# craftman22/medane_tchakorom_ufc_thesis_repository

Measured on AMD Instinct MI355X. Metric: DOF-updates/s on 3D 7-pt Poisson GMRES; achieved HBM GB/s vs peak, 1/2/4/8 GPU, higher is better.
Workload: dtype f64

## Files before the change

### medane_tchakorom_ufc_thesis_repository_amd/csrc/msplit_kernels.h

```cpp
#pragma once

#include <hip/hip_runtime.h>

#include <cstdint>

#define MSK_MAX_GROUP 32
#define MSK_DBR_CHUNK 4096

enum { MSK_SET = 0, MSK_COPY, MSK_SCALE, MSK_AXPY, MSK_AYPX, MSK_WAXPY_P1, MSK_WAXPY_M1, MSK_WAXPY };

struct Vecs {
  const double* p[MSK_MAX_GROUP];
  const double* base;
  int64_t stride;
  const double* scale;
};
struct Coefs {
  double a[MSK_MAX_GROUP];
};
struct EllOp {
  const uint8_t* code8;
  const int32_t* ddelta;
  const double* dval;
  int ndict;
// ... 11 lines not shown
  MSK_TUNE_SPMV_TEMPORAL = 2,
  MSK_TUNE_SPMV_XCD = 4,
  MSK_TUNE_SPMV_STAGE1 = 8,
  MSK_TUNE_VEC_TEMPORAL = 16,
  MSK_TUNE_MAXPY_TEMPORAL_ST = 64,
  MSK_TUNE_GM_UNFUSED = 128,
  MSK_TUNE_MAXPY_HALVES = 256,
  MSK_TUNE_SPMV_ZCHUNK = 512,
  MSK_TUNE_MDOT_SINGLE = 1024,
  MSK_TUNE_GM_SPMV_MDOT = 2048,
  MSK_TUNE_SPMV_MDOT_G2 = 4096,
  MSK_TUNE_DV_RPL1 = 8192,
  MSK_TUNE_DV_RPL2 = 16384,
  MSK_TUNE_DV_NOELL = 32768,
  MSK_TUNE_GM_OPFUSE = 65536,
  MSK_TUNE_MAXPY_UNROLL1 = 131072,
  MSK_TUNE_MDOT_UNROLL2 = 262144,
  MSK_TUNE_ELL_TEMPORAL_Y = 1048576,
  MSK_TUNE_SPMV_NTY = 2097152,
  MSK_TUNE_SPMV_REG_STAGE = 4194304,
  MSK_TUNE_DENSE_G1 = 8388608,
  MSK_TUNE_DENSE_G2 = 16777216,
  MSK_TUNE_DENSE_TEMPORAL_ST = 33554432,
  MSK_TUNE_ELL_XCD_ON = 67108864,
  MSK_TUNE_ELL_XCD_OFF = 134217728,
  MSK_TUNE_ELL_MARCH_OFF = 268435456,
  MSK_TUNE_ELL_MARCH_NOXCD = 536870912,
  MSK_TUNE_GM_BOX_MDOT_OFF = 1073741824,
  MSK_TUNE_BOX_MDOT_NOXCD = 524288,
  MSK_TUNE_BOX_MDOT_FLAT = 32
};

extern "C" {
void msk_set_tuning(int flags);
int msk_get_tuning(void);
void msk_set_spmv_group(int gb);
void msk_set_march_z(int z);
void msk_set_march_lines(int l);
int msk_dot_stage1_op(const EllOp* op, const Vecs* V, int nv, int64_t n, double* partial, int64_t nchunks,
                      const int* stop, hipStream_t s);
int msk_maxpy_op(const EllOp* op, double* wout, const Vecs* V, int nv, const double* adev, int64_t n,
                 double* partial, const int* stop, hipStream_t s);
int msk_dot_stage1(const double* w, const Vecs* V, int nv, int64_t n, double* partial, int64_t nchunks, int self,
                   const int* stop, hipStream_t s);
int msk_dot_stage2(const double* partial, int64_t nchunks, int nv, double* out, const int* stop, hipStream_t s);
int msk_seq_stage1(const double* w, const Vecs* V, int nv, int64_t n, int self, double* partial, int64_t nchunks,
                   const int* stop, hipStream_t s);
int msk_maxpy_chunk(const double* win, double* wout, const Vecs* V, int nv, const int* nvdev, const Coefs* A,
                    const double* adev, int negate, int64_t n, int accum, double* partial, const int* stop,
                    hipStream_t s);
int msk_maxpy_mdot(const double* win, double* wout, const Vecs* V, int nv, const double* adev, int64_t n,
                   double* partial, int64_t nchunks, const int* stop, hipStream_t s);
int msk_spmv(int32_t nrows, const int32_t* rowptr, const int32_t* col, const double* val, const double* x,
             const double* b, double* y, int32_t lds_cap, int mode, const double* sdev, double* vout,
             const int* stop, int64_t plane, hipStream_t s);
int msk_spmv_dv(int32_t nrows, const int32_t* rowptr, const uint8_t* len8, const uint8_t* code8,
                const int32_t* ddelta, const double* dval, int ndict, int32_t max_block, int ell_w,
                const double* x, const double* b, double* y, int mode, const double* sdev, double* vout,
                const int* stop, int64_t plane, hipStream_t s);
int msk_box_march_pick(int32_t nx, int32_t ny, int32_t nz);
int msk_march_mask(int32_t nrows, int d2, const uint8_t* code8, uint8_t* mask, hipStream_t s);
int msk_march_check(int32_t nrows, int32_t nx, int32_t ny, int d2, const uint8_t* mask, int* fail, hipStream_t s);
int msk_spmv_box_march(int32_t nx, int32_t ny, int32_t nz, int d2, const uint8_t* mask, const double* dval,
                       const double* x, const double* b, double* y, int mode, const double* sdev, double* vout,
                       const int* stop, hipStream_t s);
int msk_march_chunk_fits(int32_t nx, int32_t ny, int d2);
int msk_box_march_halo_fits(int32_t nx, int32_t ny, int32_t nz, int halo, const double *x, const double *b,
                            const double *y, int mode);
int msk_box_march_halo(int32_t nx, int32_t ny, int32_t nz, int halo, const uint8_t* mask, const double* dval,
                       const double* x, const double* b, double* y, int mode, hipStream_t s);
int msk_box_march_chunk_rv(int32_t nx, int32_t ny, int32_t nz, const uint8_t* mask, const double* rv, int64_t rvs,
                           const double* x, const double* b, double* y, int mode, const double* sdev, double* vout,
                           const int* stop, hipStream_t s);
int msk_box_spmv_mdot_rv(int32_t nx, int64_t P, int64_t n, int d2, const uint8_t* mask, const double* dval,
                         const double* rv, int64_t rvs, const double* x, const double* sdev, double* y, const Vecs* V,
                         int nv, double* partial, int64_t nchunks, const int* stop, int* self_out, hipStream_t s);
int msk_box_spmv_mdot(int32_t nx, int64_t P, int64_t n, int d2, const uint8_t* mask, const double* dval,
                      const double* x, const double* sdev, double* y, const Vecs* V, int nv, double* partial,
                      int64_t nchunks, const int* stop, int* self_out, hipStream_t s);
void msk_set_gm_wfree(int on);
int msk_get_gm_wfree(void);
void msk_set_maxpy_prefetch(int mode);
int msk_get_maxpy_prefetch(void);
int msk_box_wfree_fits(int32_t nx, int64_t P, int64_t n, int d2);
int msk_box_maxpy_march(int32_t nx, int64_t P, int64_t n, int d2, const uint8_t* mask, const double* dval, const double* x,
                        const double* sdev, double* wout, const Vecs* V, int nv, const double* adev, double* partial,
                        const int* stop, hipStream_t s);
int msk_spmm_ell(int32_t nrows, int W, const uint8_t* code8, const int32_t* ddelta, const double* dval, int ndict,
                 const double* S, int64_t lds, int nc, double* R, int64_t ldr, hipStream_t s);
int msk_spmm_ell_f32(int32_t nrows, int W, const uint8_t* code8, const int32_t* ddelta, const double* dval, int ndict,
                     const double* S, int64_t lds, int nc, float* R, int64_t ldr, hipStream_t s);
int msk_ell_encode(int32_t nrows, int W, const int32_t* rowptr, const int32_t* col, const double* val, int ndict,
                   const int32_t* ddelta, const double* dval, uint8_t* code8, int* fail, hipStream_t s);
int msk_dv_encode(int32_t nrows, const int32_t* rowptr, const int32_t* col, const double* val, int ndict,
                  const int32_t* ddelta, const double* dval, uint8_t* len8, uint8_t* code8, int* fail,
                  hipStream_t s);
int msk_spmv_mdot(int32_t nrows, const int32_t* rowptr, const int32_t* col, const double* val, const double* x,
                  const double* sdev, double* y, int32_t lds_cap, const Vecs* V, int nv, double* partial,
                  int64_t nchunks, const int* stop, hipStream_t s);
int msk_spmm(int32_t nrows, const int32_t* rowptr, const int32_t* col, const double* val, const double* S,
             int64_t lds, int nc, double* R, int64_t ldr, int32_t lds_cap, hipStream_t s);
int msk_spmm_f32(int32_t nrows, const int32_t* rowptr, const int32_t* col, const double* val, const double* S,
                 int64_t lds, int nc, float* R, int64_t ldr, int32_t lds_cap, hipStream_t s);
int msk_spmv_rows(int32_t nlisted, const int32_t* row_ids, const int32_t* rowptr, const int32_t* col,
                  const double* val, const double* x, const double* b, double* y, int resid, hipStream_t s);
int msk_stencil_spmv(int dim, int32_t nx, int32_t ny, int32_t nz, int64_t nrows, int lo, int hi, const BoxCoef* cf,
                     const double* x, const double* b, double* y, int mode, const double* sdev, double* vout,
                     const int* stop, hipStream_t s);
int msk_box_stencil(int dim, int32_t nx, int32_t ny, int32_t nz, int64_t nrows, int lo, int hi, const BoxCoef* cf,
                    int32_t* rowptr, int32_t* col, double* val, hipStream_t s);
int msk_blas1(int op, double* y, const double* x, const double* z, double alpha, int64_t n, hipStream_t s);
#define MSK_CB_MAX_GROUP 32
int msk_cb_round_store(const double* r, double* cur, float* v0, int64_t n, double* partial, const int* stop,
                       hipStream_t s);
int msk_cb_mdot(const double* w, const float* vb, int64_t stride, const double* scale, int nv, int64_t n,
                double* partial, int64_t nchunks, const int* stop, hipStream_t s);
int msk_cb_maxpy_norm(const double* win, double* cur, float* vout, const float* vb, int64_t stride,
                      const double* scale, const double* adev, int nv, int64_t n, double* partial, const int* stop,
                      hipStream_t s);
int msk_cb_accum(double* x, const int* nvdev, const float* vb, int64_t stride, const double* scale,
                 const double* coef, int64_t n, const int* stop, hipStream_t s);
int msk_cb16_round_store(const double* r, double* cur, int16_t* v0, int32_t* e0, int64_t n, double* partial,
                         const int* stop, hipStream_t s);
int msk_cb16_mdot(const double* w, const int16_t* vb, int64_t stride, const int32_t* eb, const double* scale, int nv,
                  int64_t n, double* partial, int64_t nchunks, const int* stop, hipStream_t s);
int msk_cb16_maxpy_norm(const double* win, double* cur, int16_t* vout, int32_t* eout, const int16_t* vb,
                        int64_t stride, const int32_t* eb, const double* scale, const double* adev, int nv, int64_t n,
                        double* partial, const int* stop, hipStream_t s);
int msk_cb16_accum(double* x, const int* nvdev, const int16_t* vb, int64_t stride, const int32_t* eb,
                   const double* scale, const double* coef, int64_t n, const int* stop, hipStream_t s);
int msk_pcj_diag(const int32_t* rowptr, const int32_t* col, const double* val, int32_t n, double* out, int invert,
                 hipStream_t s);
int msk_pcj_apply_norm(const double* r, const double* dinv, double* z, int64_t n, double* partial, const int* stop,
                       hipStream_t s);
int msk_pcj_mdot(const double* w, const double* dinv, const double* vb, int64_t stride, const double* scale, int nv,
                 int64_t n, double* partial, int64_t nchunks, const int* stop, hipStream_t s);
int msk_pcj_maxpy_norm(const double* win, const double* dinv, double* vout, const double* vb, int64_t stride,
                       const double* scale, const double* adev, int nv, int64_t n, double* partial, const int* stop,
                       hipStream_t s);
int msk_csr32_pack(int64_t nnz, const int32_t* col, const double* val, void* pk, unsigned int* over, hipStream_t s);
int msk_spmv_p32(int32_t nrows, const int32_t* rowptr, const void* pk, const double* x, double* y, int32_t lds_cap,
                 const double* sdev, const int* stop, int64_t plane, hipStream_t s);
}
```

### medane_tchakorom_ufc_thesis_repository_amd/csrc/msplit_kernels.hip

```cpp
#include <hip/hip_runtime.h>

#include <algorithm>
#include <cstdint>

#include "msplit_kernels.h"
#include "msplit_kdev.hpp"


namespace msk {
namespace {

template <bool NT, int SU>
__device__ __forceinline__ void stage_csr_block(int t, int32_t n2, int32_t n4, const double2* __restrict__ v2,
                                                const int4* __restrict__ c4, double* sval, int32_t* scol) {
  if constexpr (SU == 0) {
    const int lane = t & 63, w = t >> 6;
    for (int32_t ib = w * 64; ib < n2; ib += kT)
      glds16<NT>(v2 + min(ib + lane, n2 - 1), reinterpret_cast<char*>(sval) + (size_t)ib * 16);
    for (int32_t ib = w * 64; ib < n4; ib += kT)
      glds16<NT>(c4 + min(ib + lane, n4 - 1), reinterpret_cast<char*>(scol) + (size_t)ib * 16);
  } else if constexpr (SU == 1) {
    for (int32_t i = t; i < n2; i += kT) reinterpret_cast<double2*>(sval)[i] = NT ? ld_nt(v2 + i) : v2[i];
    for (int32_t i = t; i < n4; i += kT) reinterpret_cast<int4*>(scol)[i] = NT ? ld_nt(c4 + i) : c4[i];
  } else {
// ... 1047 lines not shown
  } else {
    for (int i = t; i < wlen; i += kT) {
      const int64_t r = lo + i;
      sx[i] = r >= 0 && r < n ? x[r] : 0.0;
    }
  }
  const double sc = *sdev;
  double v[7];
  march_values<D2>(dval, v);
  uint32_t m[2 * kIters];
  double xm[2 * kIters], xp[2 * kIters];
#pragma unroll
  for (int j = 0; j < kIters; ++j) {
#pragma unroll
    for (int q = 0; q < 2; ++q) {
      const int64_t r = base + j * (2 * kT) + q;
      const uint32_t mr = r < n ? (uint32_t)mask[r] : 0u;
      m[2 * j + q] = mr;
      xm[2 * j + q] = (mr & 1u) ? x[r - P] : 0.0;
      xp[2 * j + q] = (mr & 64u) ? x[r + P] : 0.0;
    }
  }
  __syncthreads();
  double wr[2 * kIters];
#pragma unroll
  for (int j = 0; j < kIters; ++j) {
#pragma unroll
    for (int q = 0; q < 2; ++q) {
      const int e = j * (2 * kT) + 2 * t + q + nx;
      const uint32_t mr = m[2 * j + q];
      const double xq[7] = {xm[2 * j + q], sx[e - nx], sx[e - 1], sx[e], sx[e + 1], sx[e + nx], xp[2 * j + q]};
      double s = 0.0;
#pragma unroll
      for (int k = 0; k < 7; ++k)
        if (mr & (1u << k)) s = s + v[k] * (xq[k] * sc);
      wr[2 * j + q] = s;
    }
    const int64_t r = base + j * (2 * kT);
    if (!y) continue;
    if (full) {
      if constexpr (NTY) {
        dx2 o;
        o.x = wr[2 * j];
        o.y = wr[2 * j + 1];
        __builtin_nontemporal_store(o, reinterpret_cast<dx2*>(y + r));
      } else {
        *reinterpret_cast<double2*>(y + r) = make_double2(wr[2 * j], wr[2 * j + 1]);
      }
    } else {
      if (r < n) y[r] = wr[2 * j];
      if (r + 1 < n) y[r + 1] = wr[2 * j + 1];
    }
  }
  if (full) {
    int g = 0;
#pragma unroll 1
    for (; g + 4 <= nv; g += 4) dot_group_full<4, VAR>(wr, V, base, 0, nv, g, red, lane, wv);
    switch (nv - g) {
      case 3: dot_group_full<3, VAR>(wr, V, base, 0, nv, g, red, lane, wv); break;
      case 2: dot_group_full<2, VAR>(wr, V, base, 0, nv, g, red, lane, wv); break;
      case 1: dot_group_full<1, VAR>(wr, V, base, 0, nv, g, red, lane, wv); break;
      default: break;
    }
  } else {
#pragma unroll 1
    for (int vi = 0; vi < nv; ++vi) {
      const double* __restrict__ yv = vec_at(V, vi);
      const double sv = vec_scale(V, vi);
      double acc = 0.0;
#pragma unroll
      for (int j = 0; j < kIters; ++j) {
        const int64_t e = base + j * (2 * kT);
        if (e < n) acc = acc + wr[2 * j] * (yv[e] * sv);
        if (e + 1 < n) acc = acc + wr[2 * j + 1] * (yv[e + 1] * sv);
      }
      acc = wave_butterfly(acc);
      if (lane == 0) red[vi][wv] = acc;
    }
  }
  __syncthreads();
  if (t < nv) partial[t * nchunks + c] = (red[t][0] + red[t][1]) + (red[t][2] + red[t][3]);
}

template <int VAR, bool NTY, int RV, int RVP = kIters>
__global__ __launch_bounds__(kT) void k_box_spmv_mdot_march(int32_t nx, int64_t P, int32_t nz, int32_t zt, int xcd,
                                                            const uint8_t* __restrict__ mask,
                                                            const double* __restrict__ dval,
                                                            const double* __restrict__ rv, int64_t rvs,
                                                            const double* __restrict__ x,
                                                            const double* __restrict__ sdev, double* __restrict__ y,
                                                            Vecs V, int nv, int self, double* __restrict__ partial,
                                                            int64_t nchunks, const int* __restrict__ stop) {
  if (stopped(stop)) return;
  extern __shared__ __attribute__((aligned(16))) char smem[];
  double* sx = reinterpret_cast<double*>(smem);
  __shared__ double red[MSK_MAX_GROUP][4];
  const int t = threadIdx.x, lane = t & 63, wv = t >> 6;
  const int64_t cpp = P / kChunk;
  int64_t tile, zg;
  if (xcd & 1) {
    const int64_t per = cpp / 8, slot = blockIdx.x / 8;
    tile = (blockIdx.x % 8) * per + slot % per;
    zg = slot / per;
  } else {
    tile = blockIdx.x % cpp;
    zg = blockIdx.x / cpp;
  }
  if (xcd & 2) zg = (nz + zt - 1) / zt - 1 - zg;
  const int32_t z0 = (int32_t)zg * zt, z1 = min(z0 + zt, nz);
  const bool down = RV != 2 && (xcd & 4) && (zg & 1);
  const double sc = *sdev;
  double v[7];
  if constexpr (!RV) march_values<false>(dval, v);
  const int nh = nx / 2;
  double xm[2 * kIters], xc[2 * kIters], xp[2 * kIters];
  double* sux = sx + kChunk + 2 * nx;
  double* suy = sux + kChunk + nx;
  double uzm[RV == 2 ? 2 * kIters : 1];
  if constexpr (RV == 2) {
    const int64_t cb = ((int64_t)z0 - 1) * P + tile * kChunk;
#pragma unroll
    for (int j = 0; j < kIters; ++j) {
      const double2 u = z0 > 0 ? ld_nt(rvs_pair(rv, cb, 3, j, t)) : make_double2(0.0, 0.0);
      uzm[2 * j] = u.x;
      uzm[2 * j + 1] = u.y;
    }
  }
  {
    const int32_t zf = down ? z1 - 1 : z0;
    const bool hasm = down ? z1 < nz : z0 > 0;
    const int64_t b0 = (int64_t)zf * P + tile * kChunk + 2 * t, bm = b0 + (down ? P : -P);
#pragma unroll
    for (int j = 0; j < kIters; ++j) {
      const double2 a = *reinterpret_cast<const double2*>(x + b0 + j * (2 * kT));
      xc[2 * j] = a.x;
      xc[2 * j + 1] = a.y;
      if (hasm) {
        const double2 m2 = *reinterpret_cast<const double2*>(x + bm + j * (2 * kT));
        xm[2 * j] = m2.x;
        xm[2 * j + 1] = m2.y;
      } else {
        xm[2 * j] = xm[2 * j + 1] = 0.0;
      }
    }
  }
  for (int32_t zi = 0; zi < z1 - z0; ++zi) {
    const int32_t z = down ? z1 - 1 - zi : z0 + zi;
    const int64_t c = (int64_t)z * cpp + tile, c0 = c * kChunk, base = c0 + 2 * t;
    const bool hasp = down ? z > 0 : z + 1 < nz;
    const int64_t dp = down ? -P : P;
    uint32_t m[kIters];
#pragma unroll
    for (int j = 0; j < kIters; ++j) {
      if (hasp) {
        const double2 p2 = *reinterpret_cast<const double2*>(x + base + dp + j * (2 * kT));
        xp[2 * j] = p2.x;
        xp[2 * j + 1] = p2.y;
      } else {
        xp[2 * j] = xp[2 * j + 1] = 0.0;
      }
      m[j] = *reinterpret_cast<const uint16_t*>(mask + base + j * (2 * kT));
    }
    double2 rqa[RV == 1 ? kIters : 1][7];
    SymTile st;
    if constexpr (RV == 2) sym_load(st, rv, c0, nx, t);
    if constexpr (RV == 1) {
#pragma unroll
      for (int j = 0; j < RVP; ++j)
#pragma unroll
        for (int k = 0; k < 7; ++k) rqa[j][k] = ld_nt(rv_pair(rv, rvs, c0, k, j, t));
    }
    double2 hl = make_double2(0.0, 0.0), hh = make_double2(0.0, 0.0);
    const bool hasl = t < nh && c0 - nx >= 0, hash = t < nh && c0 + kChunk + nx <= (int64_t)nz * P;
    if (hasl) hl = *reinterpret_cast<const double2*>(x + c0 - nx + 2 * t);
    if (hash) hh = *reinterpret_cast<const double2*>(x + c0 + kChunk + 2 * t);
    __syncthreads();
#pragma unroll
    for (int j = 0; j < kIters; ++j)
      *reinterpret_cast<double2*>(sx + nx + j * (2 * kT) + 2 * t) = make_double2(xc[2 * j], xc[2 * j + 1]);
// ... 268 lines not shown
    sv[q] = vec_scale(V, g + q);
  }
#pragma unroll
  for (int j = 0; j < kIters; ++j) {
    double p0[G], p1[G];
#pragma unroll
    for (int q = 0; q < G; ++q) {
      if (SELF && q == G - 1) {
        p0[q] = xs[2 * j] * sv[q];
        p1[q] = xs[2 * j + 1] * sv[q];
      } else {
        const double2* pv = reinterpret_cast<const double2*>(vp[q] + base + j * (2 * kT));
        const double2 v = (VAR & 1) ? ld_nt(pv) : *pv;
        p0[q] = v.x * sv[q];
        p1[q] = v.y * sv[q];
      }
    }
    const double s0 = group_sum<G>(a, p0), s1 = group_sum<G>(a, p1);
    if constexpr (G == 1) {
      u[2 * j] = s0 + u[2 * j];
      u[2 * j + 1] = s1 + u[2 * j + 1];
    } else {
      u[2 * j] = u[2 * j] + s0;
      u[2 * j + 1] = u[2 * j + 1] + s1;
    }
  }
}

template <int NL, int VAR>
__device__ __forceinline__ void maxpy_group_load(double2 (&b)[4][kIters], const Vecs& V, int g, int64_t base) {
  const double* vp[NL];
#pragma unroll
  for (int q = 0; q < NL; ++q) vp[q] = vec_at(V, g + q);
#pragma unroll
  for (int j = 0; j < kIters; ++j) {
#pragma unroll
    for (int q = 0; q < NL; ++q) {
      const double2* pv = reinterpret_cast<const double2*>(vp[q] + base + j * (2 * kT));
      b[q][j] = (VAR & 1) ? ld_nt(pv) : *pv;
    }
  }
}

template <int VAR>
__device__ __forceinline__ void maxpy_group_load_one(double2 (&b)[4][kIters], const Vecs& V, int q, int64_t base) {
  const double* vp = vec_at(V, q);
#pragma unroll
  for (int j = 0; j < kIters; ++j) {
    const double2* pv = reinterpret_cast<const double2*>(vp + base + j * (2 * kT));
    b[q][j] = (VAR & 1) ? ld_nt(pv) : *pv;
  }
}

template <int G, bool SELF>
__device__ __forceinline__ void maxpy_group_apply(double (&u)[2 * kIters], const double2 (&b)[4][kIters],
                                                  const Vecs& V, const double* __restrict__ adev, int g,
                                                  const double* xs) {
  double a[G], sv[G];
#pragma unroll
  for (int q = 0; q < G; ++q) {
    a[q] = -adev[g + q];
    sv[q] = vec_scale(V, g + q);
  }
#pragma unroll
  for (int j = 0; j < kIters; ++j) {
    double p0[G], p1[G];
#pragma unroll
    for (int q = 0; q < G; ++q) {
      const double2 v = (SELF && q == G - 1) ? *reinterpret_cast<const double2*>(xs + j * (2 * kT)) : b[q][j];
      p0[q] = v.x * sv[q];
      p1[q] = v.y * sv[q];
    }
    const double s0 = group_sum<G>(a, p0), s1 = group_sum<G>(a, p1);
    if constexpr (G == 1) {
      u[2 * j] = s0 + u[2 * j];
      u[2 * j + 1] = s1 + u[2 * j + 1];
    } else {
      u[2 * j] = u[2 * j] + s0;
      u[2 * j + 1] = u[2 * j + 1] + s1;
    }
  }
}

#define MSK_LOAD_FENCE(p_)                        \
  asm volatile("" : : "v"(p_) : "memory");        \
  __builtin_amdgcn_sched_barrier(0)
template <int VAR, int NPF>
__device__ __forceinline__ void box_plane_front(int32_t nx, int64_t P, int32_t nz, int32_t z, int64_t c0,
                                                const uint8_t* __restrict__ mask, const double* __restrict__ dval,
                                                const double* __restrict__ x, const double* __restrict__ sdev,
                                                const Vecs& V, double* sx, double (&u)[2 * kIters],
                                                double2 (&ba)[4][kIters]) {
  const int t = threadIdx.x;
  const int64_t base = c0 + 2 * t;
  const int nh = nx / 2;
  const double sc = *sdev;
  double v[7];
  march_values<false>(dval, v);
  const double* own = x + base;
  dx2 xc[kIters], xm[kIters], xp[kIters];
#pragma unroll
  for (int j = 0; j < kIters; ++j) xc[j] = *reinterpret_cast<const dx2*>(own + j * (2 * kT));
  const bool hasl = t < nh && c0 - nx >= 0, hash = t < nh && c0 + kChunk + nx <= (int64_t)nz * P;
  dx2 hl = *reinterpret_cast<const dx2*>(hasl ? x + c0 - nx + 2 * t : own);
  dx2 hh = *reinterpret_cast<const dx2*>(hash ? x + c0 + kChunk + 2 * t : own);
  MSK_LOAD_FENCE(own);
  const bool hasm = z > 0, hasp = z + 1 < nz;
  uint32_t m[kIters];
#pragma unroll
  for (int j = 0; j < kIters; ++j) xm[j] = *reinterpret_cast<const dx2*>(hasm ? own - P + j * (2 * kT) : own);
#pragma unroll
  for (int j = 0; j < kIters; ++j) xp[j] = *reinterpret_cast<const dx2*>(hasp ? own + P + j * (2 * kT) : own);
#pragma unroll
  for (int j = 0; j < kIters; ++j) m[j] = *reinterpret_cast<const uint16_t*>(mask + base + j * (2 * kT));
  MSK_LOAD_FENCE(own);
  if constexpr (NPF > 0) maxpy_group_load<NPF, VAR>(ba, V, 0, base);
  MSK_LOAD_FENCE(own);
  if (!hasl) hl = dx2{0.0, 0.0};
  if (!hash) hh = dx2{0.0, 0.0};
#pragma unroll
  for (int j = 0; j < kIters; ++j) {
    if (!hasm) xm[j] = dx2{0.0, 0.0};
    if (!hasp) xp[j] = dx2{0.0, 0.0};
  }
#pragma unroll
  for (int j = 0; j < kIters; ++j) *reinterpret_cast<dx2*>(sx + nx + j * (2 * kT) + 2 * t) = xc[j];
  if (t < nh) {
    *reinterpret_cast<dx2*>(sx + 2 * t) = hl;
    *reinterpret_cast<dx2*>(sx + nx + kChunk + 2 * t) = hh;
  }
  for (int i = t + kT; i < nh; i += kT) {
    *reinterpret_cast<double2*>(sx + 2 * i) =
        c0 - nx >= 0 ? *reinterpret_cast<const double2*>(x + c0 - nx + 2 * i) : make_double2(0.0, 0.0);
    *reinterpret_cast<double2*>(sx + nx + kChunk + 2 * i) =
        c0 + kChunk + nx <= (int64_t)nz * P ? *reinterpret_cast<const double2*>(x + c0 + kChunk + 2 * i)
                                            : make_double2(0.0, 0.0);
  }
  __syncthreads();
#pragma unroll
  for (int j = 0; j < kIters; ++j) {
#pragma unroll
    for (int q = 0; q < 2; ++q) {
      const int e = j * (2 * kT) + 2 * t + q + nx;
      const uint32_t mr = (m[j] >> (8 * q)) & 255u;
      const double xq[7] = {q ? xm[j].y : xm[j].x, sx[e - nx], sx[e - 1], sx[e], sx[e + 1], sx[e + nx],
                            q ? xp[j].y : xp[j].x};
      double s = 0.0;
#pragma unroll
      for (int k = 0; k < 7; ++k)
        if (mr & (1u << k)) s = s + v[k] * (xq[k] * sc);
      u[2 * j + q] = s;
    }
  }
}

#undef MSK_LOAD_FENCE
template <int VAR, bool NTY, bool WIDE>
__device__ __forceinline__ void box_maxpy_plane(int32_t nx, int64_t P, int32_t nz, int xcd,
                                                const uint8_t* __restrict__ mask, const double* __restrict__ dval,
                                                const double* __restrict__ x, const double* __restrict__ sdev,
                                                double* __restrict__ wout, const Vecs& V, int nv,
                                                const double* __restrict__ adev, double* __restrict__ partial,
                                                double* sx, double* red) {
  const int t = threadIdx.x, lane = t & 63, wv = t >> 6;
  const int64_t cpp = P / kChunk;
  int64_t tile, zg;
  if (xcd & 1) {
    const int64_t per = cpp / 8, slot = blockIdx.x / 8;
    tile = (blockIdx.x % 8) * per + slot % per;
// ... 490 lines not shown
    const int32_t k0 = rowptr[r], k1 = rowptr[r + 1];
    if (k1 - k0 > 255) {
      atomicOr(fail, 1);
      continue;
    }
    len8[r] = (uint8_t)(k1 - k0);
    for (int32_t k = k0; k < k1; ++k) {
      const int32_t d = col[k] - (int32_t)r;
      const long long bits = __double_as_longlong(val[k]);
      int j = 0;
      while (j < ndict && !(ddelta[j] == d && __double_as_longlong(dval[j]) == bits)) ++j;
      if (j == ndict) {
        atomicOr(fail, 1);
        break;
      }
      code8[k] = (uint8_t)j;
    }
  }
}

template <int OP>
__global__ __launch_bounds__(kT) void k_blas1(double* __restrict__ y, const double* __restrict__ x,
                                              const double* __restrict__ z, double alpha, int64_t n) {
  const int64_t stride = (int64_t)gridDim.x * kT;
  for (int64_t i = (int64_t)blockIdx.x * kT + threadIdx.x; i < n; i += stride) {
    double r;
    if (OP == MSK_SET) r = alpha;
    else if (OP == MSK_COPY) r = x[i];
    else if (OP == MSK_SCALE) r = y[i] * alpha;
    else if (OP == MSK_AXPY) r = y[i] + alpha * x[i];
    else if (OP == MSK_AYPX) r = x[i] + alpha * y[i];
    else if (OP == MSK_WAXPY_P1) r = z[i] + x[i];
    else if (OP == MSK_WAXPY_M1) r = z[i] - x[i];
    else r = z[i] + alpha * x[i];
    y[i] = r;
  }
}

}
}

using namespace msk;

__attribute__((visibility("hidden"))) int msk_tuning_flags = 0;
__attribute__((visibility("hidden"))) int msk_spmv_gb_override = 0;
__attribute__((visibility("hidden"))) int msk_march_z_override = 0;
__attribute__((visibility("hidden"))) int msk_march_lines_override = 0;
extern "C" void msk_set_tuning(int flags) { msk_tuning_flags = flags; }
extern "C" int msk_get_tuning(void) { return msk_tuning_flags; }
__attribute__((visibility("hidden"))) int msk_shape_epoch = 0;
extern "C" void msk_set_spmv_group(int gb) {
  msk_spmv_gb_override = gb;
  ++msk_shape_epoch;
}
extern "C" void msk_set_march_z(int z) {
  msk_march_z_override = z;
  ++msk_shape_epoch;
}
extern "C" void msk_set_march_lines(int l) {
  msk_march_lines_override = l;
  ++msk_shape_epoch;
}
extern "C" int msk_get_shape_epoch(void) { return msk_shape_epoch; }
__attribute__((visibility("hidden"))) int msk_gm_wfree = [] {
  const char* e = getenv("MSPLIT_GM_WFREE");
  return e ? (atoi(e) ? 1 : 0) : 1;
}();
extern "C" void msk_set_gm_wfree(int on) {
  msk_gm_wfree = on ? 1 : 0;
  ++msk_shape_epoch;
}
extern "C" int msk_get_gm_wfree(void) { return msk_gm_wfree; }
constexpr int kMaxpyPrefetchDefault = 1;
__attribute__((visibility("hidden"))) int msk_maxpy_prefetch = [] {
  const char* e = getenv("MSPLIT_MAXPY_PREFETCH");
  const int v = e ? atoi(e) : kMaxpyPrefetchDefault;
  return v < 0 || v > 3 ? kMaxpyPrefetchDefault : v;
}();
extern "C" void msk_set_maxpy_prefetch(int mode) {
  msk_maxpy_prefetch = mode < 0 || mode > 3 ? 0 : mode;
  ++msk_shape_epoch;
}
extern "C" int msk_get_maxpy_prefetch(void) { return msk_maxpy_prefetch; }

static inline XcdMap xcd_map(int32_t nrows, int64_t plane) {
  XcdMap m = {0, 0, 0};
  if (msk_tuning_flags & MSK_TUNE_SPMV_ZCHUNK) {
    const int32_t nblk = (nrows + kT - 1) / kT;
    if (nblk % 8 == 0) {
      m.bp = -1;
      m.np = nblk / 8;
    }
    return m;
  }
  if (!(msk_tuning_flags & MSK_TUNE_SPMV_XCD) || plane <= 0 || plane % kT || nrows % plane) return m;
  const int32_t bp = (int32_t)(plane / kT);
  int32_t gb = msk_spmv_gb_override > 0 ? msk_spmv_gb_override : std::min(bp / 8, 64);
  if (gb <= 0 || bp % gb || (bp / gb) % 8) return m;
  m.bp = bp;
  m.gb = gb;
  m.np = (int32_t)(nrows / plane);
  return m;
}

__attribute__((visibility("hidden"))) void msk_xcd_map3(int32_t nrows, int64_t plane, int32_t out[3]) {
  const XcdMap m = xcd_map(nrows, plane);
  out[0] = m.bp;
  out[1] = m.gb;
  out[2] = m.np;
}

static inline int grid_for(int64_t work, int cap) {
  int64_t g = (work + kT - 1) / kT;
  if (g < 1) g = 1;
  if (g > cap) g = cap;
  return (int)g;
}

extern "C" int msk_spmv(int32_t nrows, const int32_t* rowptr, const int32_t* col, const double* val, const double* x,
                        const double* b, double* y, int32_t lds_cap, int mode, const double* sdev, double* vout,
                        const int* stop, int64_t plane, hipStream_t s) {
  if (nrows <= 0) return 0;
  const unsigned g = (unsigned)((nrows + kT - 1) / kT);
  const XcdMap xm = xcd_map(nrows, plane);
  if (lds_cap > 0) {
    const bool tmp = (msk_tuning_flags & MSK_TUNE_SPMV_TEMPORAL) != 0, nty = (msk_tuning_flags & MSK_TUNE_SPMV_NTY) != 0;
    const bool reg = (msk_tuning_flags & MSK_TUNE_SPMV_REG_STAGE) != 0, stage1 = (msk_tuning_flags & MSK_TUNE_SPMV_STAGE1) != 0;
    const bool glds = !reg && !stage1;
    if ((tmp && nty) || (reg && stage1)) return (int)hipErrorInvalidValue;
    const bool nt = !tmp && !nty;
    const bool ntst = !tmp;
    const int32_t cap = glds ? ((lds_cap + 255) & ~255) : lds_cap;
    const size_t ldsb = (size_t)cap * 12;
#define LAUNCH_LDS8(M, POL_)                                                                                  \
  do {                                                                                                         \
    if (glds)                                                                                                  \
      k_spmv_lds8<M, POL_, 0><<<dim3(g), dim3(kT), ldsb, s>>>(nrows, rowptr, col, val, x, b, y, cap, sdev,     \
                                                               vout, stop, xm);                                \
    else if (stage1)                                                                                           \
      k_spmv_lds8<M, POL_, 1><<<dim3(g), dim3(kT), ldsb, s>>>(nrows, rowptr, col, val, x, b, y, cap, sdev,     \
                                                               vout, stop, xm);                                \
    else                                                                                                       \
      k_spmv_lds8<M, POL_, 4><<<dim3(g), dim3(kT), ldsb, s>>>(nrows, rowptr, col, val, x, b, y, cap, sdev,     \
                                                               vout, stop, xm);                                \
  } while (0)
#define LAUNCH_POL(M)                            \
  do {                                           \
    if (nt) LAUNCH_LDS8(M, 3);                   \
    else if (ntst) LAUNCH_LDS8(M, 2);            \
    else LAUNCH_LDS8(M, 0);                      \
  } while (0)
    if (mode == MSK_SPMV_RESID) LAUNCH_POL(MSK_SPMV_RESID);
    else if (mode == MSK_SPMV_SCALED) LAUNCH_POL(MSK_SPMV_SCALED);
    else LAUNCH_POL(MSK_SPMV_MULT);
#undef LAUNCH_POL
#undef LAUNCH_LDS8
  } else {
    if (mode == MSK_SPMV_RESID)
      k_spmv_direct<MSK_SPMV_RESID><<<dim3(g), dim3(kT), 0, s>>>(nrows, rowptr, col, val, x, b, y, sdev, vout, stop);
    else if (mode == MSK_SPMV_SCALED)
      k_spmv_direct<MSK_SPMV_SCALED><<<dim3(g), dim3(kT), 0, s>>>(nrows, rowptr, col, val, x, b, y, sdev, vout, stop);
    else
      k_spmv_direct<MSK_SPMV_MULT><<<dim3(g), dim3(kT), 0, s>>>(nrows, rowptr, col, val, x, b, y, sdev, vout, stop);
  }
  return (int)hipGetLastError();
}
// ... 298 lines not shown
  const size_t lds = (size_t)lds_cap * 12;
  const dim3 g((unsigned)nchunks), b(kT);
#define MSK_SMD(VAR_, GF_) \
  k_spmv_mdot<VAR_, GF_><<<g, b, lds, s>>>(nrows, rowptr, col, val, x, sdev, y, lds_cap, *V, nv, partial, nchunks, stop)
  const bool g2 = (msk_tuning_flags & MSK_TUNE_SPMV_MDOT_G2) != 0;
  if (vec_var()) { if (g2) MSK_SMD(1, 2); else MSK_SMD(1, 4); }
  else { if (g2) MSK_SMD(0, 2); else MSK_SMD(0, 4); }
#undef MSK_SMD
  return (int)hipGetLastError();
}

extern "C" int msk_box_spmv_mdot(int32_t nx, int64_t P, int64_t n, int d2, const uint8_t* mask, const double* dval,
                                 const double* x, const double* sdev, double* y, const Vecs* V, int nv, double* partial,
                                 int64_t nchunks, const int* stop, int* self_out, hipStream_t s) {
  return msk_box_spmv_mdot_rv(nx, P, n, d2, mask, dval, nullptr, 0, x, sdev, y, V, nv, partial, nchunks, stop,
                              self_out, s);
}

extern "C" int msk_box_spmv_mdot_rv(int32_t nx, int64_t P, int64_t n, int d2, const uint8_t* mask, const double* dval,
                                    const double* rv, int64_t rvs, const double* x, const double* sdev, double* y,
                                    const Vecs* V, int nv, double* partial, int64_t nchunks, const int* stop,
                                    int* self_out, hipStream_t s) {
  if (self_out) *self_out = 0;
  if (n <= 0 || nchunks <= 0) return 0;
  if (nx < 2 || nx > 2048 || P < nx || nv < 1 || nv > MSK_MAX_GROUP || dv_flags_bad()) return (int)hipErrorInvalidValue;
  if (rv && (!y || d2 || P % kChunk || n % P || (nx & 1) || (rvs < 0 && nx > 1024))) return (int)hipErrorInvalidValue;
  const size_t lds = (size_t)(kChunk + 2 * nx + (rv && rvs < 0 ? 2 * (kChunk + nx) : 0)) * sizeof(double);
  const dim3 g((unsigned)nchunks), b(kT);
  const bool nty = !(msk_tuning_flags & MSK_TUNE_ELL_TEMPORAL_Y);
  if (!d2 && P % kChunk == 0 && n % P == 0 && (nx & 1) == 0 && (rv || !(msk_tuning_flags & MSK_TUNE_BOX_MDOT_FLAT))) {
    static const int zenv = [] {
      const char* e = getenv("MSPLIT_BOXMDOT_ZT");
      return e ? atoi(e) : 0;
    }();
    const int32_t nz = (int32_t)(n / P);
    const int32_t zt = zenv > 0 ? zenv : 4;
    const int64_t grid = (P / kChunk) * ((nz + zt - 1) / zt);
    if (grid > INT32_MAX) return (int)hipErrorInvalidValue;
    static const int rev = [] {
      const char* e = getenv("MSPLIT_BOXMDOT_REV");
      return e && atoi(e) ? 2 : 0;
    }();
    const char* alte = getenv("MSPLIT_BOXMDOT_ALT");
    const int alt = alte && alte[0] == '1' ? 4 : 0;
    const int xcd =
        ((P / kChunk) % 8 == 0 && P / kChunk >= 32 && !(msk_tuning_flags & MSK_TUNE_BOX_MDOT_NOXCD)) | rev | alt;
    static const int self_env = [] {
      const char* e = getenv("MSPLIT_BOXMDOT_SELF");
      return e ? atoi(e) : 1;
    }();
    const double* last = V->base ? V->base + (int64_t)(nv - 1) * V->stride : V->p[nv - 1];
    const int self = self_env != 0 && last == x;
    if (self_out) *self_out = self;
    static const int rvp = [] {
      const char* e = getenv("MSPLIT_RV_PREFETCH");
      const int v = e ? atoi(e) : kIters;
      return v == 4 || v == 2 ? v : kIters;
    }();
#define MSK_BSMM_P(VAR_, NT_, RV_, P_)                                                                          \
  k_box_spmv_mdot_march<VAR_, NT_, RV_, P_><<<dim3((unsigned)grid), b, lds, s>>>(nx, P, nz, zt, xcd, mask, dval, rv, \
                                                                                 rvs, x, sdev, y, *V, nv, self,     \
                                                                                 partial, nchunks, stop)
#define MSK_BSMM(VAR_, NT_, RV_)                                                                              \
  do {                                                                                                        \
    if (RV_ == 1 && rvp == 4) MSK_BSMM_P(VAR_, NT_, RV_, 4);                                                  \
    else if (RV_ == 1 && rvp == 2) MSK_BSMM_P(VAR_, NT_, RV_, 2);                                             \
    else MSK_BSMM_P(VAR_, NT_, RV_, kIters);                                                                  \
  } while (0)
    const char* s2e = getenv("MSPLIT_RV_SYM2");
    const bool sym2 = !(s2e && s2e[0] == '0') && nx <= 512;
#define MSK_SYM2(VAR_, NT_)                                                                               \
  k_box_spmv_mdot_march_sym2<VAR_, NT_><<<dim3((unsigned)grid), dim3(2 * kT), lds, s>>>(                   \
      nx, P, nz, zt, xcd, mask, rv, x, sdev, y, *V, nv, self, partial, nchunks, stop)
    if (rv && rvs < 0 && sym2) {
      if (vec_var()) { if (nty) MSK_SYM2(1, true); else MSK_SYM2(1, false); }
      else { if (nty) MSK_SYM2(0, true); else MSK_SYM2(0, false); }
    } else if (rv && rvs < 0) {
      if (vec_var()) { if (nty) MSK_BSMM(1, true, 2); else MSK_BSMM(1, false, 2); }
      else { if (nty) MSK_BSMM(0, true, 2); else MSK_BSMM(0, false, 2); }
    } else if (rv) {
      if (vec_var()) { if (nty) MSK_BSMM(1, true, 1); else MSK_BSMM(1, false, 1); }
      else { if (nty) MSK_BSMM(0, true, 1); else MSK_BSMM(0, false, 1); }
    } else {
      if (vec_var()) { if (nty) MSK_BSMM(1, true, 0); else MSK_BSMM(1, false, 0); }
      else { if (nty) MSK_BSMM(0, true, 0); else MSK_BSMM(0, false, 0); }
    }
#undef MSK_SYM2
#undef MSK_BSMM
#undef MSK_BSMM_P
    return (int)hipGetLastError();
  }
#define MSK_BSM(D, VAR_, NT_) \
  k_box_spmv_mdot<D, VAR_, NT_><<<g, b, lds, s>>>(nx, P, n, mask, dval, x, sdev, y, *V, nv, partial, nchunks, stop)
#define MSK_BSM2(D)                                              \
  do {                                                           \
    if (vec_var()) { if (nty) MSK_BSM(D, 1, true); else MSK_BSM(D, 1, false); } \
    else { if (nty) MSK_BSM(D, 0, true); else MSK_BSM(D, 0, false); }           \
  } while (0)
  if (d2) MSK_BSM2(true);
  else MSK_BSM2(false);
#undef MSK_BSM2
#undef MSK_BSM
  return (int)hipGetLastError();
}

static bool box_mdot_marches(int32_t nx, int64_t P, int64_t n, int d2) {
  return !d2 && nx >= 2 && nx <= 2048 && P >= nx && P % kChunk == 0 && n > 0 && n % P == 0 && (nx & 1) == 0 &&
         !(msk_tuning_flags & MSK_TUNE_BOX_MDOT_FLAT) && !dv_flags_bad() && (n / P) <= INT32_MAX;
}

static bool box_mdot_fits(int32_t nx, int64_t P) { return nx >= 2 && nx <= 2048 && P >= nx && !dv_flags_bad(); }

extern "C" int msk_box_wfree_fits(int32_t nx, int64_t P, int64_t n, int d2) {
  return msk_gm_wfree && n > 0 && box_mdot_fits(nx, P) ? 1 : 0;
}

extern "C" int msk_box_maxpy_march(int32_t nx, int64_t P, int64_t n, int d2, const uint8_t* mask, const double* dval,
                                   const double* x, const double* sdev, double* wout, const Vecs* V, int nv,
                                   const double* adev, double* partial, const int* stop, hipStream_t s) {
  if (n <= 0) return 0;
  if (!box_mdot_fits(nx, P) || nv < 1) return (int)hipErrorInvalidValue;
  const double* last = V->base ? V->base + (int64_t)(nv - 1) * V->stride : (nv <= MSK_MAX_GROUP ? V->p[nv - 1] : nullptr);
  if (last != x) return (int)hipErrorInvalidValue;
  const bool nt = !(msk_tuning_flags & MSK_TUNE_MAXPY_TEMPORAL_ST);
  if (!box_mdot_marches(nx, P, n, d2)) {
    const int64_t nch = (n + kChunk - 1) / kChunk;
    if (nch > INT32_MAX) return (int)hipErrorInvalidValue;
    const size_t ldsu = (size_t)(kChunk + 2 * nx) * sizeof(double);
#define MSK_BMU(D_, VAR_, NT_)                                                                                      \
  k_box_maxpy<D_, VAR_, NT_><<<dim3((unsigned)nch), dim3(kT), ldsu, s>>>(nx, P, n, mask, dval, x, sdev, wout, *V, nv, \
                                                                        adev, partial, stop)
#define MSK_BMU2(D_)                                                                          \
  do {                                                                                        \
    if (vec_var()) { if (nt) MSK_BMU(D_, 1, true); else MSK_BMU(D_, 1, false); }              \
    else { if (nt) MSK_BMU(D_, 0, true); else MSK_BMU(D_, 0, false); }                        \
  } while (0)
    if (d2) MSK_BMU2(true);
    else MSK_BMU2(false);
#undef MSK_BMU2
#undef MSK_BMU
    return (int)hipGetLastError();
  }
  static const int zenv = [] {
    const char* e = getenv("MSPLIT_MAXPY_ZT");
    return e ? atoi(e) : 0;
  }();
  static const int rev_env = [] {
    const char* e = getenv("MSPLIT_MAXPY_REV");
    return e ? (atoi(e) ? 1 : 0) : -1;
  }();
  const int32_t nz = (int32_t)(n / P);
  const int32_t zt = zenv > 0 ? zenv : 1;
  const int64_t grid = (P / kChunk) * ((nz + zt - 1) / zt);
  if (grid > INT32_MAX) return (int)hipErrorInvalidValue;
  const int rev = (rev_env < 0 ? n > ((int64_t)1 << 25) : rev_env) ? 2 : 0;
  const int xcd = ((P / kChunk) % 8 == 0 && P / kChunk >= 32 && !(msk_tuning_flags & MSK_TUNE_BOX_MDOT_NOXCD)) | rev;
  const size_t lds = (size_t)(kChunk + 2 * nx) * sizeof(double);
  const bool nty = nt;
  static const int u2 = [] {
    const char* e = getenv("MSPLIT_MAXPY_MARCH_U2");
    return e ? atoi(e) : 0;
  }();
#define MSK_BMM(VAR_, NT_, PF_)                                                                              \
  k_box_maxpy_march<VAR_, NT_, PF_><<<dim3((unsigned)grid), dim3(kT), lds, s>>>(                                \
      nx, P, nz, zt, xcd, mask, dval, x, sdev, wout, *V, nv, adev, partial, stop)
#define MSK_BMM2(PF_)                                                              \
  do {                                                                             \
    if (vec_var()) { if (nty) MSK_BMM(1, true, PF_); else MSK_BMM(1, false, PF_); } \
// ... 86 lines not shown
```

Measured before the change: 23.87 billion.

## Add software-pipelined box SpMV+mdot march with prefetched next-plane and dot vectors

```diff
diff --git a/medane_tchakorom_ufc_thesis_repository_amd/csrc/msplit_kernels.h b/medane_tchakorom_ufc_thesis_repository_amd/csrc/msplit_kernels.h
--- a/medane_tchakorom_ufc_thesis_repository_amd/csrc/msplit_kernels.h
+++ b/medane_tchakorom_ufc_thesis_repository_amd/csrc/msplit_kernels.h
@@ -117,6 +117,8 @@
 int msk_get_gm_wfree(void);
 void msk_set_maxpy_prefetch(int mode);
 int msk_get_maxpy_prefetch(void);
+void msk_set_boxmdot_pipe(int mode);
+int msk_get_boxmdot_pipe(void);
 int msk_box_wfree_fits(int32_t nx, int64_t P, int64_t n, int d2);
 int msk_box_maxpy_march(int32_t nx, int64_t P, int64_t n, int d2, const uint8_t* mask, const double* dval, const double* x,
                         const double* sdev, double* wout, const Vecs* V, int nv, const double* adev, double* partial,
diff --git a/medane_tchakorom_ufc_thesis_repository_amd/csrc/msplit_kernels.hip b/medane_tchakorom_ufc_thesis_repository_amd/csrc/msplit_kernels.hip
--- a/medane_tchakorom_ufc_thesis_repository_amd/csrc/msplit_kernels.hip
+++ b/medane_tchakorom_ufc_thesis_repository_amd/csrc/msplit_kernels.hip
@@ -1153,6 +1153,202 @@
   if (t < nv) partial[t * nchunks + c] = (red[t][0] + red[t][1]) + (red[t][2] + red[t][3]);
 }
 
+#define MSK_LOAD_FENCE(p_)                        \
+  asm volatile("" : : "v"(p_) : "memory");        \
+  __builtin_amdgcn_sched_barrier(0)
+
+template <int G, int VAR>
+__device__ __forceinline__ void dot_group_issue(dx2 (&q)[4][kIters], const Vecs& V, int64_t base, int g) {
+#pragma unroll
+  for (int u = 0; u < G; ++u) {
+    const double* __restrict__ yv = vec_at(V, g + u);
+#pragma unroll
+    for (int j = 0; j < kIters; ++j) {
+      const dx2* pq = reinterpret_cast<const dx2*>(yv + base + j * (2 * kT));
+      q[u][j] = (VAR & 1) ? __builtin_nontemporal_load(pq) : *pq;
+    }
+  }
+}
+template <int G>
+__device__ __forceinline__ void dot_group_finish(const double (&wr)[2 * kIters], const dx2 (&q)[4][kIters],
+                                                 const double (&sv)[4], int g, double (*red)[4], int lane, int wv) {
+  double acc[G];
+#pragma unroll
+  for (int u = 0; u < G; ++u) {
+    acc[u] = 0.0;
+#pragma unroll
+    for (int j = 0; j < kIters; ++j) {
+      acc[u] = acc[u] + wr[2 * j] * (q[u][j].x * sv[u]);
+      acc[u] = acc[u] + wr[2 * j + 1] * (q[u][j].y * sv[u]);
+    }
+  }
+#pragma unroll
+  for (int u = 0; u < G; ++u) {
+    acc[u] = wave_butterfly(acc[u]);
+    if (lane == 0) red[g + u][wv] = acc[u];
+  }
+}
+
+template <int VAR, bool NTY, int NPF>
+__device__ __forceinline__ void box_mdot_pipe(int32_t nx, int64_t P, int32_t nz, int32_t zt, int xcd,
+                                              const uint8_t* __restrict__ mask, const double* __restrict__ dval,
+                                              const double* __restrict__ x, const double* __restrict__ sdev,
+                                              double* __restrict__ y, const Vecs& V, int nv, int self,
+                                              double* __restrict__ partial, int64_t nchunks, double* sx,
+                                              double (*red)[4]) {
+  const int t = threadIdx.x, lane = t & 63, wv = t >> 6;
+  const int64_t cpp = P / kChunk;
+  int64_t tile, zg;
+  if (xcd & 1) {
+    const int64_t per = cpp / 8, slot = blockIdx.x / 8;
+    tile = (blockIdx.x % 8) * per + slot % per;
+    zg = slot / per;
+  } else {
+    tile = blockIdx.x % cpp;
+    zg = blockIdx.x / cpp;
+  }
+  if (xcd & 2) zg = (nz + zt - 1) / zt - 1 - zg;
+  const int32_t z0 = (int32_t)zg * zt, z1 = min(z0 + zt, nz);
+  const bool down = (xcd & 4) && (zg & 1);
+  const int64_t dp = down ? -P : P, total = (int64_t)nz * P;
+  const double sc = *sdev;
+  double v[7];
+  march_values<false>(dval, v);
+  const int nh = nx / 2;
+  const dx2 zero = {0.0, 0.0};
+  dx2 xm[kIters], xc[kIters], xp[kIters], xn[kIters], hl, hh, hln, hhn;
+  uint32_t m[kIters], mn[kIters];
+  dx2 q[4][kIters];
+  double sv0[4] = {1.0, 1.0, 1.0, 1.0};
+#pragma unroll
+  for (int u = 0; u < NPF; ++u) sv0[u] = vec_scale(V, u);
+  bool hasm, hasp, hasl, hash;
+  {
+    const int32_t zf = down ? z1 - 1 : z0;
+    const int64_t c0 = (int64_t)zf * P + tile * kChunk;
+    const double* own = x + c0 + 2 * t;
+    hasm = down ? zf + 1 < nz : zf > 0;
+    hasp = down ? zf > 0 : zf + 1 < nz;
+    hasl = t < nh && c0 - nx >= 0;
+    hash = t < nh && c0 + kChunk + nx <= total;
+#pragma unroll
+    for (int j = 0; j < kIters; ++j) xc[j] = *reinterpret_cast<const dx2*>(own + j * (2 * kT));
+    hl = *reinterpret_cast<const dx2*>(hasl ? x + c0 - nx + 2 * t : own);
+    hh = *reinterpret_cast<const dx2*>(hash ? x + c0 + kChunk + 2 * t : own);
+    MSK_LOAD_FENCE(own);
+#pragma unroll
+    for (int j = 0; j < kIters; ++j) xm[j] = *reinterpret_cast<const dx2*>(hasm ? own - dp + j * (2 * kT) : own);
+#pragma unroll
+    for (int j = 0; j < kIters; ++j) xp[j] = *reinterpret_cast<const dx2*>(hasp ? own + dp + j * (2 * kT) : own);
+#pragma unroll
+    for (int j = 0; j < kIters; ++j) m[j] = *reinterpret_cast<const uint16_t*>(mask + c0 + 2 * t + j * (2 * kT));
+    MSK_LOAD_FENCE(own);
+  }
+  const int32_t np = z1 - z0;
+  for (int32_t zi = 0; zi < np; ++zi) {
+    const int32_t z = down ? z1 - 1 - zi : z0 + zi;
+    const int64_t c = (int64_t)z * cpp + tile, c0 = c * kChunk, base = c0 + 2 * t;
+    const double* own = x + base;
+    if constexpr (NPF > 0) dot_group_issue<NPF, VAR>(q, V, base, 0);
+    MSK_LOAD_FENCE(own);
+    hl = hasl ? hl : zero;
+    hh = hash ? hh : zero;
+    __syncthreads();
+#pragma unroll
+    for (int j = 0; j < kIters; ++j) *reinterpret_cast<dx2*>(sx + nx + j * (2 * kT) + 2 * t) = xc[j];
+    if (t < nh) {
+      *reinterpret_cast<dx2*>(sx + 2 * t) = hl;
+      *reinterpret_cast<dx2*>(sx + nx + kChunk + 2 * t) = hh;
+    }
+    __syncthreads();
+#pragma unroll
+    for (int j = 0; j < kIters; ++j) {
+      xm[j] = hasm ? xm[j] : zero;
+      xp[j] = hasp ? xp[j] : zero;
+    }
+    double wr[2 * kIters];
+#pragma unroll
+    for (int j = 0; j < kIters; ++j) {
+#pragma unroll
+      for (int qq = 0; qq < 2; ++qq) {
+        const int e = j * (2 * kT) + 2 * t + qq + nx;
+        const uint32_t mr = (m[j] >> (8 * qq)) & 255u;
+        const double am = qq ? xm[j].y : xm[j].x, ac = qq ? xc[j].y : xc[j].x, ap = qq ? xp[j].y : xp[j].x;
+        const double xq[7] = {down ? ap : am, sx[e - nx], sx[e - 1], ac, sx[e + 1], sx[e + nx], down ? am : ap};
+        double s = 0.0;
+#pragma unroll
+        for (int k = 0; k < 7; ++k)
+          if (mr & (1u << k)) s = s + v[k] * (xq[k] * sc);
+        wr[2 * j + qq] = s;
+      }
+    }
+    if (y) {
+#pragma unroll
+      for (int j = 0; j < kIters; ++j) {
+        dx2 o;
+        o.x = wr[2 * j];
+        o.y = wr[2 * j + 1];
+        if constexpr (NTY) __builtin_nontemporal_store(o, reinterpret_cast<dx2*>(y + base + j * (2 * kT)));
+        else *reinterpret_cast<dx2*>(y + base + j * (2 * kT)) = o;
+      }
+    }
+    const bool more = zi + 1 < np;
+    const int64_t c0n = c0 + dp;
+    const bool hasp_n = more && (down ? z - 2 >= 0 : z + 2 < nz);
+    const bool hasl_n = more && t < nh && c0n - nx >= 0, hash_n = more && t < nh && c0n + kChunk + nx <= total;
+    const uint8_t* mo = mask + base + (more ? dp : 0);
+    MSK_LOAD_FENCE(own);
+    hln = *reinterpret_cast<const dx2*>(hasl_n ? x + c0n - nx + 2 * t : own);
+    hhn = *reinterpret_cast<const dx2*>(hash_n ? x + c0n + kChunk + 2 * t : own);
+#pragma unroll
+    for (int j = 0; j < kIters; ++j)
+      xn[j] = *reinterpret_cast<const dx2*>(hasp_n ? own + 2 * dp + j * (2 * kT) : own);
+#pragma unroll
+    for (int j = 0; j < kIters; ++j) mn[j] = *reinterpret_cast<const uint16_t*>(mo + j * (2 * kT));
+    MSK_LOAD_FENCE(own);
+    if constexpr (NPF > 0) dot_group_finish<NPF>(wr, q, sv0, 0, red, lane, wv);
+    if constexpr (NPF == 4) {
+      const int nvm = nv - self;
+      int g = 4;
+#pragma unroll 1
+      for (; g + 4 <= nvm; g += 4) dot_group_full<4, VAR>(wr, V, base, 0, nv, g, red, lane, wv);
+      switch (nvm - g) {
+        case 3: dot_group_full<3, VAR>(wr, V, base, 0, nv, g, red, lane, wv); break;
+        case 2: dot_group_full<2, VAR>(wr, V, base, 0, nv, g, red, lane, wv); break;
+        case 1: dot_group_full<1, VAR>(wr, V, base, 0, nv, g, red, lane, wv); break;
+        default: break;
+      }
+    }
+    if (self) {
+      const double sv = vec_scale(V, nv - 1);
+      double acc = 0.0;
+#pragma unroll
+      for (int j = 0; j < kIters; ++j) {
+        acc = acc + wr[2 * j] * (xc[j].x * sv);
+        acc = acc + wr[2 * j + 1] * (xc[j].y * sv);
+      }
+      acc = wave_butterfly(acc);
+      if (lane == 0) red[nv - 1][wv] = acc;
+    }
+    __syncthreads();
+    if (t < nv) partial[t * nchunks + c] = (red[t][0] + red[t][1]) + (red[t][2] + red[t][3]);
+#pragma unroll
+    for (int j = 0; j < kIters; ++j) {
+      xm[j] = xc[j];
+      xc[j] = xp[j];
+      xp[j] = xn[j];
+      m[j] = mn[j];
+    }
+    hl = hln;
+    hh = hhn;
+    hasm = true;
+    hasp = hasp_n;
+    hasl = hasl_n;
+    hash = hash_n;
+  }
+}
+
+constexpr int kPipeRVP = 16;
 template <int VAR, bool NTY, int RV, int RVP = kIters>
 __global__ __launch_bounds__(kT) void k_box_spmv_mdot_march(int32_t nx, int64_t P, int32_t nz, int32_t zt, int xcd,
                                                             const uint8_t* __restrict__ mask,
@@ -1166,6 +1362,10 @@
   extern __shared__ __attribute__((aligned(16))) char smem[];
   double* sx = reinterpret_cast<double*>(smem);
   __shared__ double red[MSK_MAX_GROUP][4];
+  if constexpr (RV == 0 && RVP >= kPipeRVP) {
+    box_mdot_pipe<VAR, NTY, RVP - kPipeRVP>(nx, P, nz, zt, xcd, mask, dval, x, sdev, y, V, nv, self, partial, nchunks, sx, red);
+    return;
+  }
   const int t = threadIdx.x, lane = t & 63, wv = t >> 6;
   const int64_t cpp = P / kChunk;
   int64_t tile, zg;
@@ -1600,9 +1800,6 @@
   }
 }
 
-#define MSK_LOAD_FENCE(p_)                        \
-  asm volatile("" : : "v"(p_) : "memory");        \
-  __builtin_amdgcn_sched_barrier(0)
 template <int VAR, int NPF>
 __device__ __forceinline__ void box_plane_front(int32_t nx, int64_t P, int32_t nz, int32_t z, int64_t c0,
                                                 const uint8_t* __restrict__ mask, const double* __restrict__ dval,
@@ -2259,6 +2456,17 @@
   ++msk_shape_epoch;
 }
 extern "C" int msk_get_maxpy_prefetch(void) { return msk_maxpy_prefetch; }
+constexpr int kBoxMdotPipeDefault = 1;
+__attribute__((visibility("hidden"))) int msk_boxmdot_pipe = [] {
+  const char* e = getenv("MSPLIT_BOXMDOT_PIPE");
+  const int v = e ? atoi(e) : kBoxMdotPipeDefault;
+  return v < 0 || v > 2 ? kBoxMdotPipeDefault : v;
+}();
+extern "C" void msk_set_boxmdot_pipe(int mode) {
+  msk_boxmdot_pipe = mode < 0 || mode > 2 ? 0 : mode;
+  ++msk_shape_epoch;
+}
+extern "C" int msk_get_boxmdot_pipe(void) { return msk_boxmdot_pipe; }
 
 static inline XcdMap xcd_map(int32_t nrows, int64_t plane) {
   XcdMap m = {0, 0, 0};
@@ -2723,8 +2931,28 @@
       if (vec_var()) { if (nty) MSK_BSMM(1, true, 1); else MSK_BSMM(1, false, 1); }
       else { if (nty) MSK_BSMM(0, true, 1); else MSK_BSMM(0, false, 1); }
     } else {
-      if (vec_var()) { if (nty) MSK_BSMM(1, true, 0); else MSK_BSMM(1, false, 0); }
-      else { if (nty) MSK_BSMM(0, true, 0); else MSK_BSMM(0, false, 0); }
+      constexpr int kBoxMdotPipeFromNv = 1;
+      constexpr int kBoxMdotPlainAtStreamed = 4;
+      const int mode = nx <= 2 * kT ? msk_boxmdot_pipe : 0;
+      const bool pipe = mode == 2 || (mode == 1 && nv >= kBoxMdotPipeFromNv && nv - self != kBoxMdotPlainAtStreamed);
+      const int npf = pipe ? std::min(nv - self, 4) : -1;
+#define MSK_BSMM_V(P_)                                                                        \
+  do {                                                                                        \
+    if (vec_var()) { if (nty) MSK_BSMM_P(1, true, 0, P_); else MSK_BSMM_P(1, false, 0, P_); } \
+    else { if (nty) MSK_BSMM_P(0, true, 0, P_); else MSK_BSMM_P(0, false, 0, P_); }           \
+  } while (0)
+      switch (npf) {
+        case 0: MSK_BSMM_V(kPipeRVP + 0); break;
+        case 1: MSK_BSMM_V(kPipeRVP + 1); break;
+        case 2: MSK_BSMM_V(kPipeRVP + 2); break;
+        case 3: MSK_BSMM_V(kPipeRVP + 3); break;
+        case 4: MSK_BSMM_V(kPipeRVP + 4); break;
+        default:
+          if (vec_var()) { if (nty) MSK_BSMM(1, true, 0); else MSK_BSMM(1, false, 0); }
+          else { if (nty) MSK_BSMM(0, true, 0); else MSK_BSMM(0, false, 0); }
+          break;
+      }
+#undef MSK_BSMM_V
     }
 #undef MSK_SYM2
 #undef MSK_BSMM
```

Result: no change. 24.04 billion (median of 6 runs) (+0.7%).
